# jhbastek/PhysicsInformedDiffusionModels

Hardware: AMD Instinct MI355X
Metric: training samples/sec (UNet+PDE-residual step), 64x64 Darcy (higher is better)
Workload: dtype f32

## Files before the change

### physicsinformeddiffusionmodels_amd/csrc/k_attn.hip

```cpp
#include "pidm_launch.h"

namespace pidm {

static const int DH = 32;

__device__ __forceinline__ float fexp(float x) { return __expf(x); }

__global__ void __launch_bounds__(256) la_kstats_kernel(const float* __restrict__ qkv, int N, int HD, int nseg,
                                                        float* __restrict__ kpart, float* __restrict__ kstat) {
  __shared__ float sm[4][64], ssum[4][64];
  const int b = blockIdx.y, seg = blockIdx.z, tid = threadIdx.x, cl = tid & 63, rl = tid >> 6;
  const int j = blockIdx.x * 64 + cl;
  const int per = (N + nseg - 1) / nseg;
  const int n_lo = seg * per, n_hi = (n_lo + per < N) ? n_lo + per : N;
  float m = -3.0e38f, s = 0.f;
  if (j < HD) {
    const float* base = qkv + (size_t)b * N * 3 * HD + HD + j;
    int n = n_lo + rl;
    for (; n + 28 < n_hi; n += 32) {
      float v[8];
#pragma unroll
      for (int u = 0; u < 8; ++u) v[u] = base[(size_t)(n + 4 * u) * 3 * HD];
      float gm = v[0];
#pragma unroll
// ... 950 lines not shown
    f32x16 acc;
    for (int r = 0; r < 16; ++r) acc[r] = 0.f;
#pragma unroll
    for (int s2 = 0; s2 < 16; ++s2)
      acc = __builtin_amdgcn_mfma_f32_32x32x2f32(sdo[32 * ti + l31][2 * s2 + half], sv[32 * tj + l31][2 * s2 + half], acc, 0, 0, 0);
#pragma unroll
    for (int r = 0; r < 16; ++r) sdS_[(32 * ti + (r & 3) + 8 * (r >> 2) + 4 * half) * LS + 32 * tj + l31] = acc[r];
  }
  if (wave < 2) {
    f32x16 acc;
    for (int r = 0; r < 16; ++r) acc[r] = 0.f;
#pragma unroll 8
    for (int s2 = 0; s2 < 32; ++s2)
      acc = __builtin_amdgcn_mfma_f32_32x32x2f32(sS_[(2 * s2 + half) * LS + 32 * wave + l31], sdo[2 * s2 + half][l31], acc, 0, 0, 0);
#pragma unroll
    for (int r = 0; r < 16; ++r)
      out[((size_t)b * N + 32 * wave + (r & 3) + 8 * (r >> 2) + 4 * half) * 3 * HD + 2 * HD + h * DH + l31] = acc[r];
  }
  __syncthreads();
  {
    const int row = tid >> 2, c0 = (tid & 3) * 16;
    const float* pp = sS_ + row * LS + c0;
    float* pd = sdS_ + row * LS + c0;
    float dot = 0.f;
#pragma unroll
    for (int j = 0; j < 16; ++j) dot = fmaf(pd[j], pp[j], dot);
    dot += pidm_quad_xor1(dot);
    dot += pidm_quad_xor2(dot);
#pragma unroll
    for (int j = 0; j < 16; ++j) pd[j] = pp[j] * (pd[j] - dot);
  }
  __syncthreads();
  {
    const int t = wave & 1;
    f32x16 acc;
    for (int r = 0; r < 16; ++r) acc[r] = 0.f;
    if (wave < 2) {
#pragma unroll 8
      for (int s2 = 0; s2 < 32; ++s2)
        acc = __builtin_amdgcn_mfma_f32_32x32x2f32(sdS_[(32 * t + l31) * LS + 2 * s2 + half], sk[2 * s2 + half][l31], acc, 0, 0, 0);
    } else {
#pragma unroll 8
      for (int s2 = 0; s2 < 32; ++s2)
        acc = __builtin_amdgcn_mfma_f32_32x32x2f32(sdS_[(2 * s2 + half) * LS + 32 * t + l31], sq[2 * s2 + half][l31], acc, 0, 0, 0);
    }
    const float f = wave < 2 ? scale : 1.f;
    const size_t col = (wave < 2 ? 0 : HD) + h * DH + l31;
#pragma unroll
    for (int r = 0; r < 16; ++r)
      out[((size_t)b * N + 32 * t + (r & 3) + 8 * (r >> 2) + 4 * half) * 3 * HD + col] = acc[r] * f;
  }
}

static int la_nsplit(int N) {
  int ns = N / 512;
  if (ns < 1) ns = 1;
  if (ns > 8) ns = 8;
  return ns;
}
static int la_kseg(int N) {
  int s = N / 256;
  if (s < 1) s = 1;
  if (s > 16) s = 16;
  return s;
}
size_t la_scratch_floats(int B, int N, int heads) {
  const size_t a = (size_t)B * la_kseg(N) * heads * DH * 2, b = (size_t)B * heads * la_nsplit(N) * 1024;
  return a + b + (size_t)heads * DH * 128 + 64;
}

int launch_la_forward(const float* qkv, float* kstat, float* ctx, float* attn, float* qstat, int B, int N, int heads,
                      float* scratch, hipStream_t st) {
  const int HD = heads * DH;
  const float scale = 0.17677669529663687f;
  const int nseg = la_kseg(N), NS = la_nsplit(N);
  float* kpart = scratch;
  float* dpart = scratch + (size_t)B * nseg * HD * 2;
  hipLaunchKernelGGL(la_kstats_kernel, dim3(cdiv(HD, 64), B, nseg), dim3(256), 0, st, qkv, N, HD, nseg, kpart, nseg == 1 ? kstat : nullptr);
  PIDM_CHECK_LAUNCH("la_kstats_kernel");
  if (nseg > 1) {
    hipLaunchKernelGGL(la_kstats_final_kernel, dim3(cdiv(B * HD, 256)), dim3(256), 0, st, kpart, B, HD, nseg, kstat);
    PIDM_CHECK_LAUNCH("la_kstats_final_kernel");
  }
  hipLaunchKernelGGL(HIP_KERNEL_NAME(la_nreduce_kernel<0>), dim3(B * heads, NS), dim3(256), 0, st, qkv, kstat, nullptr, nullptr,
                     dpart, N, heads, scale, NS == 1 ? ctx : nullptr, nullptr, 1.f / (float)N);
  PIDM_CHECK_LAUNCH("la_context");
  if (NS > 1) {
    hipLaunchKernelGGL(HIP_KERNEL_NAME(la_nreduce_final_kernel<0>), dim3(B * heads), dim3(256), 0, st, dpart, nullptr, ctx, nullptr, NS,
                       1.f / (float)N);
    PIDM_CHECK_LAUNCH("la_context_final");
  }
  const size_t npix = (size_t)B * N;
  if (N % 32 == 0)
    hipLaunchKernelGGL(HIP_KERNEL_NAME(la_out_kernel<true>), dim3((unsigned)((npix + 127) / 128), (npix + 127) / 128 < 1024 ? heads : 1), dim3(256), 0, st, qkv, ctx, attn,
                       qstat, N, heads, npix, scale);
  else
    hipLaunchKernelGGL(HIP_KERNEL_NAME(la_out_kernel<false>), dim3((unsigned)((npix + 127) / 128), (npix + 127) / 128 < 1024 ? heads : 1), dim3(256), 0, st, qkv, ctx, attn,
                       qstat, N, heads, npix, scale);
  PIDM_CHECK_LAUNCH("la_out_kernel");
  return 0;
}

int launch_la_backward(const float* qkv, const float* kstat, const float* qstat, const float* ctx, const float* dA, float* dctx,
                       float* rowdot, float* dqkv, int B, int N, int heads, float* scratch, hipStream_t st) {
  const float scale = 0.17677669529663687f;
  const int NS = la_nsplit(N);
  float* dpart = scratch;
  hipLaunchKernelGGL(HIP_KERNEL_NAME(la_nreduce_kernel<1>), dim3(B * heads, NS), dim3(256), 0, st, qkv, qstat, dA, ctx, dpart, N, heads,
                     scale, NS == 1 ? dctx : nullptr, rowdot, 1.f);
  PIDM_CHECK_LAUNCH("la_dctx");
  if (NS > 1) {
    hipLaunchKernelGGL(HIP_KERNEL_NAME(la_nreduce_final_kernel<1>), dim3(B * heads), dim3(256), 0, st, dpart, ctx, dctx, rowdot, NS, 1.f);
    PIDM_CHECK_LAUNCH("la_dctx_final");
  }
  if (N % 32 == 0 && N >= 64) {
    const size_t npix = (size_t)B * N;
    int ppb = N % 128 == 0 ? 128 : (N % 64 == 0 ? 64 : 32);
    (void)npix;
    if (const char* pe = knob("PIDM_LA_PPB")) { const int v = atoi(pe); if ((v == 32 || v == 64 || v == 128) && N % v == 0) ppb = v; }
    PIDM_PROF_NAME("la_bwd_pix_mfma_kernel");
    hipLaunchKernelGGL(la_bwd_pix_mfma_kernel, dim3((unsigned)((size_t)B * N / ppb), heads), dim3(2 * ppb), 0, st, qkv, kstat, qstat, ctx,
                       dctx, rowdot, dA, dqkv, N, heads, scale, ppb);
  } else {
    hipLaunchKernelGGL(la_bwd_pix_kernel, dim3(cdiv(N, 256), B * heads), dim3(256), 0, st, qkv, kstat, qstat, ctx, dctx, rowdot,
                       dA, dqkv, N, heads, scale);
  }
  PIDM_CHECK_LAUNCH("la_bwd_pix_kernel");
  return 0;
}

bool la_fused_ok(int N, int heads, int Cout, int ld_dy) {
  const bool off = knob("PIDM_NO_LA_FUSED") != nullptr;
  return !off && N % 128 == 0 && (Cout == 32 || Cout == 64 || Cout == 128) && (ld_dy & 3) == 0 && heads >= 1 && heads <= 14;
}
int launch_la_forward_fused(const float* qkv, float* kstat, float* ctx, float* qstat, const float* w_out, const float* bias,
                            const float* resid, float* y, int Cout, int B, int N, int heads, float* scratch, hipStream_t st) {
  if (!la_fused_ok(N, heads, Cout, Cout)) return fail("fused attention forward: N=%d Cout=%d not eligible", N, Cout);
  const int HD = heads * DH;
  const float scale = 0.17677669529663687f;
  const int nseg = la_kseg(N), NS = la_nsplit(N);
  float* kpart = scratch;
  float* dpart = scratch + (size_t)B * nseg * HD * 2;
  hipLaunchKernelGGL(la_kstats_kernel, dim3(cdiv(HD, 64), B, nseg), dim3(256), 0, st, qkv, N, HD, nseg, kpart, nseg == 1 ? kstat : nullptr);
  PIDM_CHECK_LAUNCH("la_kstats_kernel");
  if (nseg > 1) {
    hipLaunchKernelGGL(la_kstats_final_kernel, dim3(cdiv(B * HD, 256)), dim3(256), 0, st, kpart, B, HD, nseg, kstat);
    PIDM_CHECK_LAUNCH("la_kstats_final_kernel");
  }
  hipLaunchKernelGGL(HIP_KERNEL_NAME(la_nreduce_kernel<0>), dim3(B * heads, NS), dim3(256), 0, st, qkv, kstat, nullptr, nullptr,
                     dpart, N, heads, scale, NS == 1 ? ctx : nullptr, nullptr, 1.f / (float)N);
  PIDM_CHECK_LAUNCH("la_context");
  if (NS > 1) {
    hipLaunchKernelGGL(HIP_KERNEL_NAME(la_nreduce_final_kernel<0>), dim3(B * heads), dim3(256), 0, st, dpart, nullptr, ctx, nullptr, NS,
                       1.f / (float)N);
    PIDM_CHECK_LAUNCH("la_context_final");
  }
  float* wt = dpart + (size_t)B * heads * NS * 1024;
  hipLaunchKernelGGL(la_wt_kernel, dim3(cdiv(Cout * HD, 256)), dim3(256), 0, st, w_out, wt, Cout, HD);
// ... 44 lines not shown
    (void)hipFuncSetAttribute(reinterpret_cast<const void*>(&la_bwd_dkdv_kernel), hipFuncAttributeMaxDynamicSharedMemorySize, 96 * 1024);
    attr_done = true;
  }
  hipLaunchKernelGGL(la_bwd_dq_kernel, gridp, dim3(256), ((size_t)heads * 1056 + 4 * 32 * kLaTileLd) * sizeof(float), st, qkv, qstat, ctx, dy, ld_dy, w_out, Cout,
                     dqkv, N, heads, scale);
  PIDM_CHECK_LAUNCH("la_bwd_dq_kernel");
  hipLaunchKernelGGL(la_bwd_dkdv_kernel, gridp, dim3(256), ((size_t)heads * kLaDkvLds + 4 * 32 * kLaTileLd) * sizeof(float), st, qkv, kstat, dctx, rowdot, dqkv, N,
                     heads);
  PIDM_CHECK_LAUNCH("la_bwd_dkdv_kernel");
  return 0;
}

int launch_mid_attn(const float* qkv, const float* dO, float* out, int B, int N, int heads, bool bwd, hipStream_t st) {
  if (N > 64) return fail("mid attention: %d tokens > 64", N);
  const float scale = 0.17677669529663687f;
  const size_t lds = ((size_t)4 * N * 33 + (size_t)2 * N * (N + 1)) * sizeof(float);
  static bool attr_done = false;
  if (!attr_done) {
    (void)hipFuncSetAttribute(reinterpret_cast<const void*>(&mid_attn_kernel<true>), hipFuncAttributeMaxDynamicSharedMemorySize, 96 * 1024);
    (void)hipFuncSetAttribute(reinterpret_cast<const void*>(&mid_attn_kernel<false>), hipFuncAttributeMaxDynamicSharedMemorySize, 96 * 1024);
    attr_done = true;
  }
  const bool mfma_off = [] { const char* e = knob("PIDM_MID_ATTN_MFMA"); return e && !atoi(e); }();
  if (N == 64 && !mfma_off) {
    static bool attr64 = false;
    if (!attr64) {
      (void)hipFuncSetAttribute(reinterpret_cast<const void*>(&mid_attn64_kernel<true>), hipFuncAttributeMaxDynamicSharedMemorySize, 96 * 1024);
      (void)hipFuncSetAttribute(reinterpret_cast<const void*>(&mid_attn64_kernel<false>), hipFuncAttributeMaxDynamicSharedMemorySize, 96 * 1024);
      attr64 = true;
    }
    if (bwd) hipLaunchKernelGGL(HIP_KERNEL_NAME(mid_attn64_kernel<true>), dim3(B * heads), dim3(256), lds, st, qkv, dO, out, heads, scale);
    else hipLaunchKernelGGL(HIP_KERNEL_NAME(mid_attn64_kernel<false>), dim3(B * heads), dim3(256), lds, st, qkv, dO, out, heads, scale);
    PIDM_CHECK_LAUNCH("mid_attn64_kernel");
    return 0;
  }
  if (bwd)
    hipLaunchKernelGGL(HIP_KERNEL_NAME(mid_attn_kernel<true>), dim3(B * heads), dim3(256), lds, st, qkv, dO, out, N, heads, scale);
  else
    hipLaunchKernelGGL(HIP_KERNEL_NAME(mid_attn_kernel<false>), dim3(B * heads), dim3(256), lds, st, qkv, dO, out, N, heads, scale);
  PIDM_CHECK_LAUNCH("mid_attn_kernel");
  return 0;
}

}

extern "C" size_t pidm_linear_attention_ws(int B, int N, int heads) {
  return ((size_t)B * heads * (1024 + 32) + pidm::la_scratch_floats(B, N, heads)) * sizeof(float);
}
extern "C" int pidm_linear_attention_forward(const float* qkv, float* out, float* kstat, float* ctx, float* qstat, int B, int N,
                                             int heads, void* workspace, void* stream) {
  if (!qkv || !out || !kstat || !ctx || !qstat || !workspace || B < 1 || N < 1 || heads < 1)
    return pidm::fail("linear attention: bad arguments");
  float* scratch = reinterpret_cast<float*>(workspace) + (size_t)B * heads * (1024 + 32);
  return pidm::launch_la_forward(qkv, kstat, ctx, out, qstat, B, N, heads, scratch, reinterpret_cast<hipStream_t>(stream));
}
extern "C" int pidm_linear_attention_backward(const float* qkv, const float* kstat, const float* qstat, const float* ctx,
                                              const float* d_out, float* dqkv, int B, int N, int heads, void* workspace,
                                              void* stream) {
  if (!qkv || !kstat || !qstat || !ctx || !d_out || !dqkv || !workspace || B < 1 || N < 1 || heads < 1)
    return pidm::fail("linear attention backward: bad arguments");
  float* dctx = reinterpret_cast<float*>(workspace);
  float* rowdot = dctx + (size_t)B * heads * 1024;
  float* scratch = rowdot + (size_t)B * heads * 32;
  return pidm::launch_la_backward(qkv, kstat, qstat, ctx, d_out, dctx, rowdot, dqkv, B, N, heads, scratch,
                                  reinterpret_cast<hipStream_t>(stream));
}
extern "C" size_t pidm_linear_attention_out_backward_ws(int B, int N, int heads, int Cout) {
  return ((size_t)B * heads * (1024 + 32) + (size_t)B * Cout * heads * 32 + pidm::la_fused_scratch_floats(B, N, heads, Cout)) *
         sizeof(float);
}
extern "C" int pidm_linear_attention_out_backward(const float* qkv, const float* kstat, const float* qstat, const float* ctx,
                                                  const float* d_y, int ld_dy, const float* w_out, int Cout, float* dqkv,
                                                  float* dw_out, int B, int N, int heads, void* workspace, void* stream) {
  if (!qkv || !kstat || !qstat || !ctx || !d_y || !w_out || !dqkv || !dw_out || !workspace || B < 1)
    return pidm::fail("fused attention backward: bad arguments");
  const int HD = heads * 32;
  float* dctx = reinterpret_cast<float*>(workspace);
  float* rowdot = dctx + (size_t)B * heads * 1024;
  float* dwpart = rowdot + (size_t)B * heads * 32;
  float* scratch = dwpart + (size_t)B * Cout * HD;
  hipStream_t st = reinterpret_cast<hipStream_t>(stream);
  if (pidm::launch_la_backward_fused(qkv, kstat, qstat, ctx, d_y, ld_dy, w_out, Cout, dctx, rowdot, dqkv, dwpart, B, N, heads,
                                     scratch, st))
    return -1;
  return pidm::launch_split_reduce(dwpart, dw_out, nullptr, nullptr, B, Cout, HD, 1, Cout, HD, st);
}
extern "C" int pidm_linear_attention_out_forward(const float* qkv, const float* w_out, const float* bias, const float* residual,
                                                 float* y, int Cout, float* kstat, float* ctx, float* qstat, int B, int N,
                                                 int heads, void* workspace, void* stream) {
  if (!qkv || !w_out || !y || !kstat || !ctx || !qstat || !workspace || B < 1) return pidm::fail("fused attention forward: bad arguments");
  float* scratch = reinterpret_cast<float*>(workspace) + (size_t)B * heads * (1024 + 32);
  return pidm::launch_la_forward_fused(qkv, kstat, ctx, qstat, w_out, bias, residual, y, Cout, B, N, heads, scratch,
                                       reinterpret_cast<hipStream_t>(stream));
}
```

### physicsinformeddiffusionmodels_amd/csrc/pidm_launch.h

```cpp
#pragma once
#include <vector>

#include "pidm_common.h"

namespace pidm {
struct ReduceQueue {
  std::vector<ReduceDesc> v;
  unsigned nblocks = 0;
  void push(const float* src, float* dst, const float* bsrc, float* bdst, size_t sstride, int nsplit, int M, int N, int T,
            int MP, int NP) {
    ReduceDesc d{};
    d.src = src; d.dst = dst; d.bsrc = bsrc; d.bdst = bdst; d.sstride = sstride;
    d.nsplit = nsplit; d.M = M; d.N = N; d.T = T; d.MP = MP; d.NP = NP;
    const size_t total = (size_t)M * N * T + (bdst ? M : 0);
    const size_t flat = (size_t)MP * T * NP;
    d.blk0 = nblocks;
    d.mode = (nsplit <= 8 && T <= 16 && (size_t)M * N * T >= 32768) ? 1 : 0;
    if (d.mode == 0 && nsplit > 8 && flat >= 4096 && (flat & 3) == 0 && (sstride & 3) == 0 && (reinterpret_cast<size_t>(src) & 15) == 0) {
      d.mode = 2;
      d.bsrc = nullptr;
      d.bdst = nullptr;
      d.nblk = (unsigned)((flat / 4 + 31) / 32);
      nblocks += d.nblk;
      v.push_back(d);
// ... 70 lines not shown
bool conv_nt4_ok(const ConvGeom& g, int KC);
int launch_conv_rs(const ConvGeom& g, const float* src0, const float* src1, const unsigned short* wsplit, const float* bias,
                   const float* residual, float* out, hipStream_t st);
int launch_conv_fp32(const ConvGeom& g, const float* src0, const float* src1, const float* wp, const float* bias, const float* residual,
                     float* out, int sigmoid_last, hipStream_t st, int KC, int NT, bool nt4);
size_t packed_floats(const ConvGeom& g);
int packed_kp(const ConvGeom& g);
int launch_pack(const ConvGeom& g, int kind, const float* w_ref, float* w_packed, int srcKH, int srcKW, int n_off, int k_off,
                int n_src, int k_src, hipStream_t st);
unsigned make_pack_desc(const ConvGeom& g, int kind, const float* w_ref, float* w_packed, int srcKH, int srcKW, int n_off,
                        int k_off, int n_src, int k_src, PackDesc* d);
int launch_pack_multi(const PackDesc* table_dev, int ndesc, unsigned nblocks, hipStream_t st);
int launch_conv(const ConvGeom& g, const float* src0, const float* src1, const float* wp, const float* bias,
                const float* residual, float* out, int sigmoid_last, hipStream_t st);
size_t smallm_splitk_ws_floats(int M, int N, int K);
bool smallm_splitk_ok(int M, int N, int K, int lda, int ldw);
int launch_smallm_splitk(const float* A, int lda, const float* W, int ldw, float* out, int M, int N, int K, float* scratch, hipStream_t st);
size_t wgrad_ws_bytes(const ConvGeom& g);
int launch_wgrad(const ConvGeom& g, const float* src0, const float* src1, const float* dy, int ld_dy, float* dw_ref,
                 float* dbias, void* workspace, hipStream_t st, ReduceQueue* defer = nullptr, WgradQueue* wq = nullptr);
bool launch_wgrad_rs(const WgradGeom& plan, const float* src0, const float* src1, const float* dy, int ld_dy, float* partial,
                     float* bias_partial, hipStream_t st, WgradGeom* used, WgradQueue* wq = nullptr);
bool wgrad_rs_queueable(const ConvGeom& g, const float* src0, const float* dy, int ld_dy);
bool wgrad_rs4_eligible(const ConvGeom& g, int ld_dy);
bool launch_wgrad_rs4(const WgradGeom& plan, const float* src0, const float* src1, const float* dy, int ld_dy, float* partial,
                      float* bias_partial, hipStream_t st, WgradGeom* used, WgradQueue* wq = nullptr);
bool launch_wgrad_rs7(const WgradGeom& plan, const float* src0, const float* dy, int ld_dy, float* partial, float* bias_partial,
                      hipStream_t st, WgradGeom* used);
size_t colsum_ws_bytes(size_t rows, int C);
int launch_colsum(const float* x, size_t rows, int C, int ld, float* out, void* workspace, hipStream_t st,
                  ReduceQueue* defer = nullptr);
size_t gn_ws_bytes(int B, int HW, int C, int G);
int launch_gn_stats(const float* x, int B, int HW, int C, int G, float* stats, void* ws, hipStream_t st);
bool gn_apply_ln_ok(int C);
int launch_gn_apply(const float* x, float* stats, const float* gamma, const float* beta, const float* ss, const float* ssb,
                    int ldss, const float* res, float* y, int B, int HW, int C, int G, void* ws, hipStream_t st, int part_chunks = 0,
                    const float* ln_gamma = nullptr, float* ln_out = nullptr);
int launch_gn_bwd(const float* x, const float* dy, const float* stats, const float* gamma, const float* beta, const float* ss,
                  const float* ssb, int ldss, float* dss, float* dx, float* dgamma, float* dbeta, int B, int HW, int C, int G,
                  void* ws, hipStream_t st, float* dgb_persist = nullptr, ReduceQueue* defer = nullptr, int part_chunks = 0);
int launch_layernorm_fwd(const float* x, const float* gamma, float* y, size_t npix, int C, hipStream_t st);
size_t layernorm_bwd_ws_bytes(int C);
int layernorm_bwd_gn_chunks(int B, int HW);
int launch_layernorm_bwd(const float* x, const float* gamma, const float* dy, const float* res, float* dx, float* dgamma,
                         size_t npix, int C, void* ws, hipStream_t st, ReduceQueue* defer = nullptr, float* res_colsum = nullptr,
                         const float* gn_x = nullptr, const float* gn_stats = nullptr, const float* gn_gamma = nullptr,
                         const float* gn_beta = nullptr, int gn_G = 0, int gn_B = 0, int gn_HW = 0, void* gn_part = nullptr);
int launch_act_fwd(const float* x, float* y, size_t n, int act, hipStream_t st);
int launch_act_bwd(const float* x, const float* dy, float* dx, size_t n, int act, hipStream_t st);
int launch_sinusoid(const int64_t* t, float* emb, int B, int dim, hipStream_t st);
int launch_copy_add(float* dst, int ldd, const float* a, int lda, const float* b, int ldb, size_t rows, int cols, hipStream_t st);
int launch_nchw_to_nhwc(const float* src, float* dst, int B, int C, int HW, const float* y_sig, hipStream_t st);
size_t la_scratch_floats(int B, int N, int heads);
int launch_la_forward(const float* qkv, float* kstat, float* ctx, float* attn, float* qstat, int B, int N, int heads,
                      float* scratch, hipStream_t st);
bool la_fused_ok(int N, int heads, int Cout, int ld_dy);
bool la_fused_pays(int B, int N);
size_t la_fused_scratch_floats(int B, int N, int heads, int Cout);
int launch_la_forward_fused(const float* qkv, float* kstat, float* ctx, float* qstat, const float* w_out, const float* bias,
                            const float* resid, float* y, int Cout, int B, int N, int heads, float* scratch, hipStream_t st);
int launch_la_backward_fused(const float* qkv, const float* kstat, const float* qstat, const float* ctx, const float* dy, int ld_dy,
                             const float* w_out, int Cout, float* dctx, float* rowdot, float* dqkv, float* dwpart, int B, int N,
                             int heads, float* scratch, hipStream_t st);
int launch_la_backward(const float* qkv, const float* kstat, const float* qstat, const float* ctx, const float* dA, float* dctx,
                       float* rowdot, float* dqkv, int B, int N, int heads, float* scratch, hipStream_t st);
bool lap_ok(int N, int heads, int C, int Cout);
size_t lap_scratch_floats(int B, int N, int heads, int C);
size_t lap_saved_floats(int B, int heads, int C);
size_t lap_dw_ranges(int N, int C);
size_t lap_bwd_tmp_floats(int B, int heads, int C);
int launch_lap_forward(const float* xn, const float* wqkv, const float* wout, const float* bias, const float* resid, float* y,
                       float* saved, float* qstat, int C, int B, int N, int heads, float* scratch, hipStream_t st);
int launch_lap_backward(const float* xn, const float* dy, const float* wqkv, const float* wout, const float* saved, const float* qstat,
                        float* dxn, float* dwqk_part, float* dwv_part, float* dwout_part, float* tmp, int C, int B, int N, int heads,
                        float* scratch, hipStream_t st);
int launch_mid_attn(const float* qkv, const float* dO, float* out, int B, int N, int heads, bool bwd, hipStream_t st);
}
```

### physicsinformeddiffusionmodels_amd/csrc/unet_engine.hip

```cpp
#include <map>
#include <string>
#include <vector>

#include <stdlib.h>

#include "pidm_launch.h"

extern char** environ;

namespace pidm {

struct Arena {
  char* base = nullptr;
  size_t off = 0, hwm = 0, cap = 0;
  bool dry = false;
  float* alloc(size_t nfloats) {
    off = align_up(off, 256);
    char* p = base + off;
    off += nfloats * sizeof(float);
    if (off > hwm) hwm = off;
    return reinterpret_cast<float*>(p);
  }
  size_t mark() const { return off; }
  void release(size_t m) { off = m; }
  bool overflow() const { return !dry && hwm > cap; }
};

struct ConvLayer {
  int w = -1, b = -1;
  int C0 = 0, C1 = 0, Cout = 0, K = 1, stride = 1, pad = 0, transposed = 0, H = 1;
  size_t off_f = 0, off_d = 0;
  bool dgrad = true;
  int pad_mode = 0;
};

struct ResBlock {
  ConvLayer c1, c2, cr;
  bool has_mlp = false, has_res = false;
  int C0 = 0, C1 = 0, Co = 0, H = 0;
  int gn1w = -1, gn1b = -1, gn2w = -1, gn2b = -1, mlpw = -1, mlpb = -1;
  int ss_off = 0;
  const float *x0 = nullptr, *x1 = nullptr;
  float *a = nullptr, *st1 = nullptr, *bact = nullptr, *c = nullptr, *st2 = nullptr;
};

struct AttnBlock {
  bool mid = false;
  int C = 0, H = 0, gamma = -1;
  ConvLayer qkv, out;
  const float* x = nullptr;
  float *xn = nullptr, *qkvb = nullptr, *kstat = nullptr, *qstat = nullptr, *ctx = nullptr, *attn = nullptr;
  bool xn_ready = false;
  float* out_pre = nullptr;
  size_t mk_pre = 0;
  float* lsaved = nullptr;
  bool projected = false;
};

struct GraphSeg {
  hipGraph_t graph = nullptr;
  hipGraphExec_t exec = nullptr;
  hipEvent_t ev_after = nullptr;
  long long kernels = 0;
};
struct TapeState {
  std::vector<ResBlock> rb;
  std::vector<AttnBlock> attn;
  std::vector<const float*> skip, down_in, up_in;
  int tape_B = 0;
  const float* x_in = nullptr;
  float *emb = nullptr, *h1 = nullptr, *h1g = nullptr, *temb = nullptr, *st = nullptr, *ss = nullptr, *h0 = nullptr, *xfinal = nullptr;
  const float* out_nchw = nullptr;
  bool tape_cond = false;
  const float* cond_in = nullptr;
  float *e1 = nullptr, *e1g = nullptr, *e2 = nullptr, *h0pre = nullptr;
  int plan_B = 0;
  size_t plan_tape_b = 0, plan_tmp_b = 0, plan_defer_b = 0;
};
struct GraphEntry {
  std::vector<uint64_t> key;
  std::vector<GraphSeg> segs;
  TapeState tape;
  const void* red_dev = nullptr;
  uint64_t stamp = 0;
};
struct GraphCapture {
  GraphEntry* entry = nullptr;
  hipStream_t user_st = nullptr;
  bool open = false, failed = false;
  long long kernels0 = 0;
};
static const size_t kMaxGraphs = 6;
static const size_t kMaxSeenKeys = 16;
static long long g_graph_launches = 0, g_graph_kernels = 0, g_graph_captures = 0;
static void graph_entry_free(GraphEntry& e) {
  for (auto& sg : e.segs) {
    if (sg.exec) (void)hipGraphExecDestroy(sg.exec);
    if (sg.graph) (void)hipGraphDestroy(sg.graph);
  }
  e.segs.clear();
}

}

using namespace pidm;

struct pidm_unet {
  pidm_unet_cfg cfg;
  std::vector<std::string> names;
// ... 578 lines not shown
         7919L * (wgrad_group_on(1, 1, false) ? 1 : 0) +
         104729L * (knob("PIDM_WGRAD_GROUP_MAXWORK") ? atol(knob("PIDM_WGRAD_GROUP_MAXWORK")) % 65521 : 0) +
         15485863L * (knob("PIDM_LAP_NPER_DIV") ? atol(knob("PIDM_LAP_NPER_DIV")) % 8 : 0);
}
static bool attn_shape_projectable(const AttnBlock& a, int heads) { return !a.mid && a.out.b >= 0 && lap_ok(a.H * a.H, heads, a.C, a.C); }
static bool attn_projected(const AttnBlock& a, int heads) {
  bool off; int min_n;
  lap_knobs(&off, &min_n);
  return !off && a.H * a.H >= min_n && attn_shape_projectable(a, heads);
}

static int attn_fwd(Run& r, AttnBlock& a, const float* x, float** out_p) {
  pidm_unet* U = r.U;
  const int B = r.B, N = a.H * a.H, C = a.C, heads = U->heads, HD = heads * 32;
  const size_t npix = (size_t)B * N;
  float* out = a.xn_ready ? a.out_pre : act_alloc(r, npix * C);
  const size_t mk = a.xn_ready ? a.mk_pre : r.tmp.mark();
  a.x = x;
  if (!a.xn_ready) {
    a.xn = act_alloc(r, npix * C);
    RUN(launch_layernorm_fwd(x, U->P[a.gamma], a.xn, npix, C, r.st));
  }
  a.xn_ready = false;
  a.projected = attn_projected(a, heads);
  if (a.projected) {
    a.qkvb = nullptr;
    a.lsaved = act_alloc(r, lap_saved_floats(B, heads, C));
    a.qstat = act_alloc(r, npix * heads * 2);
    RUN(launch_lap_forward(a.xn, U->P[a.qkv.w], U->P[a.out.w], U->P[a.out.b], x, out, a.lsaved, a.qstat, C, B, N, heads, r.scratch, r.st));
    r.tmp.release(mk);
    *out_p = out;
    return 0;
  }
  a.qkvb = act_alloc(r, npix * 3 * HD);
  if (conv_fwd(r, a.qkv, a.xn, nullptr, nullptr, a.qkvb)) return -1;
  if (!a.mid && (la_fused_ok(N, heads, C, C) && la_fused_pays(B, N))) {
    a.attn = nullptr;
    a.kstat = act_alloc(r, (size_t)B * HD * 2);
    a.ctx = act_alloc(r, (size_t)B * heads * 1024);
    a.qstat = act_alloc(r, npix * heads * 2);
    RUN(launch_la_forward_fused(a.qkvb, a.kstat, a.ctx, a.qstat, U->P[a.out.w], a.out.b >= 0 ? U->P[a.out.b] : nullptr, x, out, C, B,
                                N, heads, r.scratch, r.st));
    r.tmp.release(mk);
    *out_p = out;
    return 0;
  }
  a.attn = act_alloc(r, npix * HD);
  if (a.mid) {
    RUN(launch_mid_attn(a.qkvb, nullptr, a.attn, B, N, heads, false, r.st));
  } else {
    a.kstat = act_alloc(r, (size_t)B * HD * 2);
    a.ctx = act_alloc(r, (size_t)B * heads * 1024);
    a.qstat = act_alloc(r, npix * heads * 2);
    RUN(launch_la_forward(a.qkvb, a.kstat, a.ctx, a.attn, a.qstat, B, N, heads, r.scratch, r.st));
  }
  if (conv_fwd(r, a.out, a.attn, nullptr, x, out)) return -1;
  r.tmp.release(mk);
  *out_p = out;
  return 0;
}

static int forward_impl(Run& r, const float* x_nhwc, const int64_t* t, float* out_nchw, const float* cond_nhwc) {
  pidm_unet* U = r.U;
  const int B = r.B, P = U->cfg.image_size, dim = U->cfg.dim, n = U->n_lv, td = U->tdim;
  U->tape_B = B;
  U->x_in = x_nhwc;
  U->out_nchw = out_nchw;
  U->emb = act_alloc(r, (size_t)B * dim);
  RUN(launch_sinusoid(t, U->emb, B, dim, r.st));
  U->h1 = act_alloc(r, (size_t)B * td);
  if (conv_fwd(r, U->lin1, U->emb, nullptr, nullptr, U->h1)) return -1;
  U->h1g = act_alloc(r, (size_t)B * td);
  RUN(launch_act_fwd(U->h1, U->h1g, (size_t)B * td, 1, r.st));
  U->temb = act_alloc(r, (size_t)B * td);
  if (conv_fwd(r, U->lin2, U->h1g, nullptr, nullptr, U->temb)) return -1;
  U->st = act_alloc(r, (size_t)B * td);
  RUN(launch_act_fwd(U->temb, U->st, (size_t)B * td, 0, r.st));
  U->ss = act_alloc(r, (size_t)B * U->ss_total);
  if (conv_fwd(r, U->lincat, U->st, nullptr, nullptr, U->ss)) return -1;

  U->h0 = act_alloc(r, (size_t)B * P * P * dim);
  if (conv_fwd(r, U->init_conv, x_nhwc, nullptr, nullptr, U->h0)) return -1;
  U->tape_cond = cond_nhwc != nullptr;
  if (cond_nhwc) {
    const size_t nh = (size_t)B * P * P * dim;
    U->cond_in = cond_nhwc;
    U->h0pre = U->h0;
    U->e1 = act_alloc(r, nh);
    if (conv_fwd(r, U->emb1, cond_nhwc, nullptr, nullptr, U->e1)) return -1;
    U->e1g = act_alloc(r, nh);
    RUN(launch_act_fwd(U->e1, U->e1g, nh, 1, r.st));
    U->e2 = act_alloc(r, nh);
    if (conv_fwd(r, U->emb2, U->e1g, nullptr, nullptr, U->e2)) return -1;
    float* hc = act_alloc(r, nh);
    if (conv_fwd(r, U->comb, U->h0pre, U->e2, nullptr, hc)) return -1;
    U->h0 = hc;
  }
  float* x = U->h0;
  int irb = 0, iat = 0;
  for (int i = 0; i < n; ++i) {
    if (resblock_fwd(r, U->rb[irb++], x, nullptr, &x)) return -1;
    if (resblock_fwd(r, U->rb[irb++], x, nullptr, &x, &U->attn[iat])) return -1;
    if (attn_fwd(r, U->attn[iat++], x, &x)) return -1;
    U->skip[i] = x;
    if (i < n - 1) {
      U->down_in[i] = x;
      const int Ho = out_h(U->down[i]);
// ... 220 lines not shown
  if (r.dry ? attn_projected(a, heads) : a.projected) {
    const size_t nr = (size_t)B * lap_dw_ranges(N, C);
    const size_t n_qk = nr * 2 * HD * C, n_v = (size_t)B * HD * C, n_o = (size_t)B * C * HD;
    float* dwqk = r.defer_on ? r.defer.alloc(n_qk) : r.tmp.alloc(n_qk);
    float* dwv = r.defer_on ? r.defer.alloc(n_v) : r.tmp.alloc(n_v);
    float* dwo = r.defer_on ? r.defer.alloc(n_o) : r.tmp.alloc(n_o);
    float* ltmp = r.tmp.alloc(lap_bwd_tmp_floats(B, heads, C));
    g_xn = r.tmp.alloc(npix * C);
    RUN(launch_lap_backward(a.xn, g_out, U->P[a.qkv.w], U->P[a.out.w], a.lsaved, a.qstat, g_xn, dwqk, dwv, dwo, ltmp, C, B, N, heads, r.scratch,
                            r.st));
    if (U->have_grads && !r.dry) {
      float* gw = U->G[a.qkv.w];
      if (r.q()) {
        r.q()->push(dwqk, gw, nullptr, nullptr, (size_t)2 * HD * C, (int)nr, 2 * HD, C, 1, 2 * HD, C);
        r.q()->push(dwv, gw + (size_t)2 * HD * C, nullptr, nullptr, (size_t)HD * C, B, HD, C, 1, HD, C);
        r.q()->push(dwo, U->G[a.out.w], nullptr, nullptr, (size_t)C * HD, B, C, HD, 1, C, HD);
      } else {
        RUN(launch_split_reduce(dwqk, gw, nullptr, nullptr, (int)nr, 2 * HD, C, 1, 2 * HD, C, r.st));
        RUN(launch_split_reduce(dwv, gw + (size_t)2 * HD * C, nullptr, nullptr, B, HD, C, 1, HD, C, r.st));
        RUN(launch_split_reduce(dwo, U->G[a.out.w], nullptr, nullptr, B, C, HD, 1, C, HD, r.st));
      }
    }
    float* ln_part = r.part_alloc(layernorm_bwd_ws_bytes(C) + colsum_ws_bytes(1024, C));
    RUN(launch_layernorm_bwd(a.x, U->P[a.gamma], g_xn, g_out, g_x, U->G[a.gamma], npix, C, ln_part, r.st, r.q(),
                             (U->have_grads && !r.dry) ? U->G[a.out.b] : nullptr, gn_x, gn_st, gn_gm, gn_bt, U->groups, B, N, gn_part));
    if (pc_prev) *pc_prev = gn_pc;
    if (!r.keep_frames()) r.tmp.release(mk);
    return 0;
  }
  if (!a.mid && (la_fused_ok(N, heads, C, C) && la_fused_pays(B, N))) {
    g_qkv = r.tmp.alloc(npix * 3 * HD);
    float* dctx = r.tmp.alloc((size_t)B * heads * 1024);
    float* rowdot = r.tmp.alloc((size_t)B * heads * 32);
    const size_t dwn = (size_t)B * C * HD;
    float* dwpart = r.defer_on ? r.defer.alloc(dwn) : r.tmp.alloc(dwn);
    RUN(launch_la_backward_fused(a.qkvb, a.kstat, a.qstat, a.ctx, g_out, C, U->P[a.out.w], C, dctx, rowdot, g_qkv, dwpart, B, N,
                                 heads, r.scratch, r.st));
    if (U->have_grads && !r.dry) {
      if (r.q()) r.q()->push(dwpart, U->G[a.out.w], nullptr, nullptr, (size_t)C * HD, B, C, HD, 1, C, HD);
      else RUN(launch_split_reduce(dwpart, U->G[a.out.w], nullptr, nullptr, B, C, HD, 1, C, HD, r.st));
      if (a.out.b >= 0) out_bias_with_ln = true;
    }
    g_xn = r.tmp.alloc(npix * C);
  } else {
    if (conv_wgrad(r, a.out, a.attn, nullptr, g_out)) return -1;
    float* g_attn = r.tmp.alloc(npix * HD);
    if (conv_dgrad(r, a.out, g_out, nullptr, g_attn)) return -1;
    g_qkv = r.tmp.alloc(npix * 3 * HD);
    if (a.mid) {
      RUN(launch_mid_attn(a.qkvb, g_attn, g_qkv, B, N, heads, true, r.st));
    } else {
      float* dctx = r.tmp.alloc((size_t)B * heads * 1024);
      float* rowdot = r.tmp.alloc((size_t)B * heads * 32);
      RUN(launch_la_backward(a.qkvb, a.kstat, a.qstat, a.ctx, g_attn, dctx, rowdot, g_qkv, B, N, heads, r.scratch, r.st));
    }
    g_xn = g_attn;
    if (C > HD) g_xn = r.tmp.alloc(npix * C);
  }
  if (conv_wgrad(r, a.qkv, a.xn, nullptr, g_qkv)) return -1;
  if (conv_dgrad(r, a.qkv, g_qkv, nullptr, g_xn)) return -1;
  float* ln_part = r.part_alloc(layernorm_bwd_ws_bytes(C) + colsum_ws_bytes(1024, C));
  RUN(launch_layernorm_bwd(a.x, U->P[a.gamma], g_xn, g_out, g_x, U->G[a.gamma], npix, C, ln_part, r.st, r.q(),
                           out_bias_with_ln ? U->G[a.out.b] : nullptr, gn_x, gn_st, gn_gm, gn_bt, U->groups, B, N, gn_part));
  if (pc_prev) *pc_prev = gn_pc;
  if (!r.keep_frames()) r.tmp.release(mk);
  return 0;
}

static size_t scratch_floats_needed(pidm_unet* U, int B) {
  size_t mx = 1 << 16;
  auto upd = [&](size_t bytes) { if (bytes / 4 + 64 > mx) mx = bytes / 4 + 64; };
  auto conv_ws = [&](const ConvLayer& L) {
    ConvGeom g;
    if (L.transposed) {
      if (geom_wgrad_transposed(L, B, L.Cout, &g)) return;
    } else if (geom_fwd_layer(L, B, 0, &g)) {
      return;
    }
    upd(wgrad_ws_bytes(g));
    const int Ho = out_h(L);
    upd(colsum_ws_bytes((size_t)B * Ho * Ho, L.Cout));
  };
  conv_ws(U->init_conv); conv_ws(U->lin1); conv_ws(U->lin2); conv_ws(U->lincat); conv_ws(U->final_conv);
  for (auto& m : U->rb) {
    conv_ws(m.c1); conv_ws(m.c2);
    if (m.has_res) conv_ws(m.cr);
    upd(gn_ws_bytes(B, m.H * m.H, m.Co, U->groups));
  }
  for (auto& a : U->attn) {
    conv_ws(a.qkv); conv_ws(a.out);
    upd(layernorm_bwd_ws_bytes(a.C) + colsum_ws_bytes(1024, a.C));
    upd(la_scratch_floats(B, a.H * a.H, U->heads) * sizeof(float));
    if (attn_shape_projectable(a, U->heads)) upd(lap_scratch_floats(B, a.H * a.H, U->heads, a.C) * sizeof(float));
    if (!a.mid && la_fused_ok(a.H * a.H, U->heads, a.C, a.C) && la_fused_pays(B, a.H * a.H)) upd(la_fused_scratch_floats(B, a.H * a.H, U->heads, a.C) * sizeof(float));
  }
  for (int i = 0; i < U->n_lv - 1; ++i) { conv_ws(U->down[i]); conv_ws(U->up[i]); }
  return mx;
}

static int cap_begin(Run& r) {
  GraphCapture* c = r.cap;
  if (hipStreamBeginCapture(r.st, hipStreamCaptureModeThreadLocal) != hipSuccess) {
    (void)hipGetLastError();
    c->failed = true;
    return fail("graph capture: hipStreamBeginCapture failed");
  }
  c->open = true;
// ... 676 lines not shown
```

Baseline: 8228.

## Add single-block-per-head linear attention forward and backward kernels for small N

```diff
diff --git a/physicsinformeddiffusionmodels_amd/csrc/k_attn.hip b/physicsinformeddiffusionmodels_amd/csrc/k_attn.hip
--- a/physicsinformeddiffusionmodels_amd/csrc/k_attn.hip
+++ b/physicsinformeddiffusionmodels_amd/csrc/k_attn.hip
@@ -1026,6 +1026,255 @@
   }
 }
 
+template <int NT>
+__global__ void __launch_bounds__(256) la_one_fwd_kernel(const float* __restrict__ qkv, float* __restrict__ out,
+                                                         float* __restrict__ kstat, float* __restrict__ ctx,
+                                                         float* __restrict__ qstat, int heads, float scale) {
+  constexpr int N = 32 * NT, PW = 4 * NT;
+  __shared__ float red[4][1024], sc[32][33], smax[4][32];
+  __shared__ double ssum[8][32];
+  const int bh = blockIdx.x, b = bh / heads, h = bh % heads, HD = heads * DH;
+  const int tid = threadIdx.x, lane = tid & 63, half = lane >> 5, l31 = lane & 31;
+  const int wave = __builtin_amdgcn_readfirstlane(tid >> 6);
+  const float* q0 = qkv + (size_t)b * N * 3 * HD + h * DH;
+  float kx[PW], vx[PW];
+  {
+    const float* kp = q0 + (size_t)(wave * 2 * PW + half) * 3 * HD + HD + l31;
+#pragma unroll
+    for (int j = 0; j < PW; ++j) {
+      kx[j] = kp[(size_t)(2 * j) * 3 * HD];
+      vx[j] = kp[(size_t)(2 * j) * 3 * HD + HD];
+    }
+  }
+  f32x4 qn[4] = {};
+  if (wave < NT) {
+    const float* qp = q0 + (size_t)(32 * wave + l31) * 3 * HD + 16 * half;
+#pragma unroll
+    for (int k = 0; k < 4; ++k) qn[k] = *reinterpret_cast<const f32x4*>(qp + 4 * k);
+  }
+  float m = kx[0];
+#pragma unroll
+  for (int j = 1; j < PW; ++j) m = fmaxf(m, kx[j]);
+  m = fmaxf(m, pidm_other_half(m));
+  if (half == 0) smax[wave][l31] = m;
+  __syncthreads();
+  const float cm = fmaxf(fmaxf(smax[0][l31], smax[1][l31]), fmaxf(smax[2][l31], smax[3][l31]));
+  double s = 0.0;
+#pragma unroll
+  for (int j = 0; j < PW; ++j) {
+    kx[j] = fexp(kx[j] - cm);
+    s += (double)kx[j];
+  }
+  ssum[2 * wave + half][l31] = s;
+  __syncthreads();
+  double S = ssum[0][l31];
+#pragma unroll
+  for (int w = 1; w < 8; ++w) S += ssum[w][l31];
+  const float cis = 1.f / (float)S;
+  if (wave == 0 && half == 0) {
+    kstat[((size_t)b * HD + h * DH + l31) * 2] = cm;
+    kstat[((size_t)b * HD + h * DH + l31) * 2 + 1] = cis;
+  }
+  f32x16 acc;
+  for (int r = 0; r < 16; ++r) acc[r] = 0.f;
+#pragma unroll
+  for (int j = 0; j < PW; ++j) acc = __builtin_amdgcn_mfma_f32_32x32x2f32(kx[j] * cis, vx[j], acc, 0, 0, 0);
+#pragma unroll
+  for (int r = 0; r < 16; ++r) red[wave][((r & 3) + 8 * (r >> 2) + 4 * half) * 32 + l31] = acc[r];
+  __syncthreads();
+  {
+    const float alpha = 1.f / (float)N;
+#pragma unroll
+    for (int k = 0; k < 4; ++k) {
+      const int e = tid + 256 * k;
+      const float v = ((red[0][e] + red[1][e]) + (red[2][e] + red[3][e])) * alpha;
+      ctx[(size_t)bh * 1024 + e] = v;
+      sc[e >> 5][e & 31] = v;
+    }
+  }
+  __syncthreads();
+  for (int t = wave; t < NT; t += 4) {
+    float qv[16];
+#pragma unroll
+    for (int k = 0; k < 4; ++k) { qv[4 * k] = qn[k][0]; qv[4 * k + 1] = qn[k][1]; qv[4 * k + 2] = qn[k][2]; qv[4 * k + 3] = qn[k][3]; }
+    if (t + 4 < NT) {
+      const float* qp = q0 + (size_t)(32 * (t + 4) + l31) * 3 * HD + 16 * half;
+#pragma unroll
+      for (int k = 0; k < 4; ++k) qn[k] = *reinterpret_cast<const f32x4*>(qp + 4 * k);
+    }
+    float qm = qv[0];
+#pragma unroll
+    for (int k = 1; k < 16; ++k) qm = fmaxf(qm, qv[k]);
+    qm = fmaxf(qm, pidm_other_half(qm));
+    float qs = 0.f;
+#pragma unroll
+    for (int k = 0; k < 16; ++k) {
+      qv[k] = fexp(qv[k] - qm);
+      qs += qv[k];
+    }
+    qs += pidm_other_half(qs);
+    const float inv = 1.f / qs;
+    const size_t p = (size_t)b * N + 32 * t + l31;
+    if (half == 0) *reinterpret_cast<float2*>(qstat + (p * heads + h) * 2) = make_float2(qm, inv);
+    f32x16 o;
+    for (int r = 0; r < 16; ++r) o[r] = 0.f;
+#pragma unroll
+    for (int s2 = 0; s2 < 16; ++s2) o = __builtin_amdgcn_mfma_f32_32x32x2f32(qv[s2] * inv * scale, sc[16 * half + s2][l31], o, 0, 0, 0);
+    float* ob = out + ((size_t)b * N + 32 * t) * HD + h * DH + l31;
+#pragma unroll
+    for (int r = 0; r < 16; ++r) ob[(size_t)((r & 3) + 8 * (r >> 2) + 4 * half) * HD] = o[r];
+  }
+}
+
+static const int kLaOneLd = 33;
+static size_t la_one_bwd_lds(int N) { return ((size_t)4 * N * kLaOneLd + 2 * 32 * kLaOneLd + 4096 + 32) * sizeof(float); }
+
+template <int UNR>
+__device__ __forceinline__ void la_one_stage(const float* __restrict__ qrow, const float* __restrict__ drow,
+                                             const float* __restrict__ srow, int HD, int heads, int lq, int ld, int ls, float km,
+                                             float kis, float scale, float* __restrict__ sq, float* __restrict__ sp,
+                                             float* __restrict__ sv, float* __restrict__ sda, int lo, f32x16& acc) {
+  float qa[UNR], ka[UNR], va[UNR], da[UNR];
+  float2 st[UNR];
+#pragma unroll
+  for (int u = 0; u < UNR; ++u) {
+    const float* r = qrow + (size_t)(2 * u) * 3 * HD;
+    qa[u] = r[lq];
+    ka[u] = r[lq + HD];
+    va[u] = r[lq + 2 * HD];
+    da[u] = (drow + (size_t)(2 * u) * HD)[ld];
+    st[u] = *reinterpret_cast<const float2*>(srow + (size_t)(2 * u) * heads * 2 + ls);
+  }
+#pragma unroll
+  for (int u = 0; u < UNR; ++u) {
+    const float qs = fexp(qa[u] - st[u].x) * st[u].y;
+    const int o = lo + 2 * u * kLaOneLd;
+    sq[o] = qs;
+    sp[o] = fexp(ka[u] - km) * kis;
+    sv[o] = va[u];
+    sda[o] = da[u];
+    acc = __builtin_amdgcn_mfma_f32_32x32x2f32(qs * scale, da[u], acc, 0, 0, 0);
+  }
+}
+
+template <int NW>
+__global__ void __launch_bounds__(64 * NW) la_one_bwd_kernel(const float* __restrict__ qkv, const float* __restrict__ kstat,
+                                                             const float* __restrict__ qstat, const float* __restrict__ ctx,
+                                                             const float* __restrict__ dA, float* __restrict__ dqkv, int N, int heads,
+                                                             float scale) {
+  HIP_DYNAMIC_SHARED(float, sm)
+  constexpr int LS = kLaOneLd, NTH = 64 * NW, EPT = 1024 / NTH;
+  float* sq = sm;
+  float* sp = sq + (size_t)N * LS;
+  float* sv = sp + (size_t)N * LS;
+  float* sda = sv + (size_t)N * LS;
+  float* sc = sda + (size_t)N * LS;
+  float* sd = sc + 32 * LS;
+  float* red = sd + 32 * LS;
+  float* srd = red + 4096;
+  const int bh = blockIdx.x, b = bh / heads, h = bh % heads, HD = heads * DH;
+  const int tid = threadIdx.x, lane = tid & 63, half = lane >> 5, l31 = lane & 31;
+  const int wave = __builtin_amdgcn_readfirstlane(tid >> 6);
+  float cv[EPT];
+#pragma unroll
+  for (int k = 0; k < EPT; ++k) cv[k] = ctx[(size_t)bh * 1024 + tid + NTH * k];
+  const float km = kstat[((size_t)b * HD + h * DH + l31) * 2], kis = kstat[((size_t)b * HD + h * DH + l31) * 2 + 1];
+  f32x16 acc;
+  for (int r = 0; r < 16; ++r) acc[r] = 0.f;
+  {
+    const int per = N / NW, n_lo = wave * per;
+    const int lq = half * 3 * HD + h * DH + l31, ld = half * HD + h * DH + l31, ls = (half * heads + h) * 2;
+    int n0 = n_lo;
+    if (NW == 8)
+      for (; n0 + 32 <= n_lo + per; n0 += 32)
+        la_one_stage<16>(qkv + ((size_t)b * N + n0) * 3 * HD, dA + ((size_t)b * N + n0) * HD, qstat + ((size_t)b * N + n0) * heads * 2, HD,
+                         heads, lq, ld, ls, km, kis, scale, sq, sp, sv, sda, (n0 + half) * LS + l31, acc);
+    for (; n0 + 16 <= n_lo + per; n0 += 16)
+      la_one_stage<8>(qkv + ((size_t)b * N + n0) * 3 * HD, dA + ((size_t)b * N + n0) * HD, qstat + ((size_t)b * N + n0) * heads * 2, HD,
+                      heads, lq, ld, ls, km, kis, scale, sq, sp, sv, sda, (n0 + half) * LS + l31, acc);
+    if (n0 < n_lo + per)
+      la_one_stage<4>(qkv + ((size_t)b * N + n0) * 3 * HD, dA + ((size_t)b * N + n0) * HD, qstat + ((size_t)b * N + n0) * heads * 2, HD,
+                      heads, lq, ld, ls, km, kis, scale, sq, sp, sv, sda, (n0 + half) * LS + l31, acc);
+  }
+  if (NW == 8) {
+    if (wave >= 4) {
+#pragma unroll
+      for (int r = 0; r < 16; ++r) red[(wave - 4) * 1024 + ((r & 3) + 8 * (r >> 2) + 4 * half) * 32 + l31] = acc[r];
+    }
+    __syncthreads();
+    if (wave < 4) {
+#pragma unroll
+      for (int r = 0; r < 16; ++r) acc[r] += red[wave * 1024 + ((r & 3) + 8 * (r >> 2) + 4 * half) * 32 + l31];
+    }
+  }
+  if (wave < 4) {
+#pragma unroll
+    for (int r = 0; r < 16; ++r) red[wave * 1024 + ((r & 3) + 8 * (r >> 2) + 4 * half) * 32 + l31] = acc[r];
+  }
+#pragma unroll
+  for (int k = 0; k < EPT; ++k) sc[((tid + NTH * k) >> 5) * LS + (tid & 31)] = cv[k];
+  __syncthreads();
+  float dv4[EPT];
+#pragma unroll
+  for (int k = 0; k < EPT; ++k) {
+    const int e = tid + NTH * k;
+    dv4[k] = (red[e] + red[1024 + e]) + (red[2048 + e] + red[3072 + e]);
+  }
+  __syncthreads();
+#pragma unroll
+  for (int k = 0; k < EPT; ++k) {
+    const int e = tid + NTH * k, o = (e >> 5) * LS + (e & 31);
+    sd[o] = dv4[k];
+    red[o] = dv4[k] * cv[k];
+  }
+  __syncthreads();
+  if (tid < 32) {
+    float sacc = 0.f;
+    for (int j = 0; j < 32; ++j) sacc += red[tid * LS + j];
+    srd[tid] = sacc;
+  }
+  __syncthreads();
+  const float invN = 1.f / (float)N, rd = srd[l31];
+  for (int it = wave, turn = 0; it < N / 16; it += NW, ++turn) {
+    const int t = it >> 1;
+    const bool part_dq = ((wave ^ (wave >> 2) ^ turn) & 1) == 0;
+    const int ra = (32 * t + l31) * LS + 16 * half;
+    float* ob = dqkv + ((size_t)b * N + 32 * t) * 3 * HD + h * DH + l31;
+    if (part_dq) {
+      f32x16 acc1;
+      for (int r = 0; r < 16; ++r) acc1[r] = 0.f;
+#pragma unroll
+      for (int s = 0; s < 16; ++s)
+        acc1 = __builtin_amdgcn_mfma_f32_32x32x2f32(sda[ra + s], sc[l31 * LS + 16 * half + s], acc1, 0, 0, 0);
+#pragma unroll
+      for (int r = 0; r < 16; ++r) {
+        const int row = (r & 3) + 8 * (r >> 2) + 4 * half;
+        const float qs = sq[(32 * t + row) * LS + l31];
+        float dot = qs * acc1[r];
+#pragma unroll
+        for (int off = 1; off < 32; off <<= 1) dot += __shfl_xor(dot, off);
+        ob[(size_t)row * 3 * HD] = scale * qs * (acc1[r] - dot);
+      }
+    } else {
+      f32x16 acc2, acc3;
+      for (int r = 0; r < 16; ++r) { acc2[r] = 0.f; acc3[r] = 0.f; }
+#pragma unroll
+      for (int s = 0; s < 16; ++s) {
+        const int kk = 16 * half + s;
+        acc2 = __builtin_amdgcn_mfma_f32_32x32x2f32(sv[ra + s], sd[l31 * LS + kk], acc2, 0, 0, 0);
+        acc3 = __builtin_amdgcn_mfma_f32_32x32x2f32(sp[ra + s], sd[kk * LS + l31], acc3, 0, 0, 0);
+      }
+#pragma unroll
+      for (int r = 0; r < 16; ++r) {
+        const int row = (r & 3) + 8 * (r >> 2) + 4 * half;
+        float* o = ob + (size_t)row * 3 * HD;
+        o[HD] = sp[(32 * t + row) * LS + l31] * (acc2[r] * invN - rd);
+        o[2 * HD] = acc3[r] * invN;
+      }
+    }
+  }
+}
+
 static int la_nsplit(int N) {
   int ns = N / 512;
   if (ns < 1) ns = 1;
@@ -1043,10 +1292,33 @@
   return a + b + (size_t)heads * DH * 128 + 64;
 }
 
+static bool la_one_pays(int B, int N) {
+  (void)B; (void)N;
+  return true;
+}
+bool la_one_on(int B, int N) {
+  const char* e = knob("PIDM_LA_ONE");
+  if (e && !atoi(e)) return false;
+  return N >= 32 && N <= 256 && N % 32 == 0 && la_one_pays(B, N);
+}
+
 int launch_la_forward(const float* qkv, float* kstat, float* ctx, float* attn, float* qstat, int B, int N, int heads,
-                      float* scratch, hipStream_t st) {
+                      float* scratch, hipStream_t st, bool one) {
   const int HD = heads * DH;
   const float scale = 0.17677669529663687f;
+  if (one) {
+    if (N < 32 || N > 256 || N % 32) return fail("one-launch attention forward: N=%d not eligible", N);
+    const dim3 grid(B * heads), blk(256);
+#define PIDM_LA_ONE_FWD(NT_) \
+  case NT_: hipLaunchKernelGGL(HIP_KERNEL_NAME(la_one_fwd_kernel<NT_>), grid, blk, 0, st, qkv, attn, kstat, ctx, qstat, heads, scale); break;
+    switch (N / 32) {
+      PIDM_LA_ONE_FWD(1) PIDM_LA_ONE_FWD(2) PIDM_LA_ONE_FWD(3) PIDM_LA_ONE_FWD(4)
+      PIDM_LA_ONE_FWD(5) PIDM_LA_ONE_FWD(6) PIDM_LA_ONE_FWD(7) PIDM_LA_ONE_FWD(8)
+    }
+#undef PIDM_LA_ONE_FWD
+    PIDM_CHECK_LAUNCH("la_one_fwd_kernel");
+    return 0;
+  }
   const int nseg = la_kseg(N), NS = la_nsplit(N);
   float* kpart = scratch;
   float* dpart = scratch + (size_t)B * nseg * HD * 2;
@@ -1076,8 +1348,28 @@
 }
 
 int launch_la_backward(const float* qkv, const float* kstat, const float* qstat, const float* ctx, const float* dA, float* dctx,
-                       float* rowdot, float* dqkv, int B, int N, int heads, float* scratch, hipStream_t st) {
+                       float* rowdot, float* dqkv, int B, int N, int heads, float* scratch, hipStream_t st, bool one) {
   const float scale = 0.17677669529663687f;
+  if (one) {
+    if (N < 32 || N > 256 || N % 32) return fail("one-launch attention backward: N=%d not eligible", N);
+    static bool attr_done = false;
+    if (!attr_done) {
+      if (hipFuncSetAttribute(reinterpret_cast<const void*>(&la_one_bwd_kernel<8>), hipFuncAttributeMaxDynamicSharedMemorySize,
+                              (int)la_one_bwd_lds(256)) != hipSuccess ||
+          hipFuncSetAttribute(reinterpret_cast<const void*>(&la_one_bwd_kernel<4>), hipFuncAttributeMaxDynamicSharedMemorySize,
+                              (int)la_one_bwd_lds(224)) != hipSuccess)
+        return fail("one-launch attention backward: %zu bytes of LDS not granted", la_one_bwd_lds(256));
+      attr_done = true;
+    }
+    if (N >= 128 && N % 64 == 0)
+      hipLaunchKernelGGL(HIP_KERNEL_NAME(la_one_bwd_kernel<8>), dim3(B * heads), dim3(512), la_one_bwd_lds(N), st, qkv, kstat, qstat, ctx,
+                         dA, dqkv, N, heads, scale);
+    else
+      hipLaunchKernelGGL(HIP_KERNEL_NAME(la_one_bwd_kernel<4>), dim3(B * heads), dim3(256), la_one_bwd_lds(N), st, qkv, kstat, qstat, ctx,
+                         dA, dqkv, N, heads, scale);
+    PIDM_CHECK_LAUNCH("la_one_bwd_kernel");
+    return 0;
+  }
   const int NS = la_nsplit(N);
   float* dpart = scratch;
   hipLaunchKernelGGL(HIP_KERNEL_NAME(la_nreduce_kernel<1>), dim3(B * heads, NS), dim3(256), 0, st, qkv, qstat, dA, ctx, dpart, N, heads,
@@ -1228,7 +1520,8 @@
   if (!qkv || !out || !kstat || !ctx || !qstat || !workspace || B < 1 || N < 1 || heads < 1)
     return pidm::fail("linear attention: bad arguments");
   float* scratch = reinterpret_cast<float*>(workspace) + (size_t)B * heads * (1024 + 32);
-  return pidm::launch_la_forward(qkv, kstat, ctx, out, qstat, B, N, heads, scratch, reinterpret_cast<hipStream_t>(stream));
+  return pidm::launch_la_forward(qkv, kstat, ctx, out, qstat, B, N, heads, scratch, reinterpret_cast<hipStream_t>(stream),
+                                 pidm::la_one_on(B, N));
 }
 extern "C" int pidm_linear_attention_backward(const float* qkv, const float* kstat, const float* qstat, const float* ctx,
                                               const float* d_out, float* dqkv, int B, int N, int heads, void* workspace,
@@ -1239,7 +1532,7 @@
   float* rowdot = dctx + (size_t)B * heads * 1024;
   float* scratch = rowdot + (size_t)B * heads * 32;
   return pidm::launch_la_backward(qkv, kstat, qstat, ctx, d_out, dctx, rowdot, dqkv, B, N, heads, scratch,
-                                  reinterpret_cast<hipStream_t>(stream));
+                                  reinterpret_cast<hipStream_t>(stream), pidm::la_one_on(B, N));
 }
 extern "C" size_t pidm_linear_attention_out_backward_ws(int B, int N, int heads, int Cout) {
   return ((size_t)B * heads * (1024 + 32) + (size_t)B * Cout * heads * 32 + pidm::la_fused_scratch_floats(B, N, heads, Cout)) *
diff --git a/physicsinformeddiffusionmodels_amd/csrc/pidm_launch.h b/physicsinformeddiffusionmodels_amd/csrc/pidm_launch.h
--- a/physicsinformeddiffusionmodels_amd/csrc/pidm_launch.h
+++ b/physicsinformeddiffusionmodels_amd/csrc/pidm_launch.h
@@ -146,8 +146,9 @@
 int launch_copy_add(float* dst, int ldd, const float* a, int lda, const float* b, int ldb, size_t rows, int cols, hipStream_t st);
 int launch_nchw_to_nhwc(const float* src, float* dst, int B, int C, int HW, const float* y_sig, hipStream_t st);
 size_t la_scratch_floats(int B, int N, int heads);
+bool la_one_on(int B, int N);
 int launch_la_forward(const float* qkv, float* kstat, float* ctx, float* attn, float* qstat, int B, int N, int heads,
-                      float* scratch, hipStream_t st);
+                      float* scratch, hipStream_t st, bool one);
 bool la_fused_ok(int N, int heads, int Cout, int ld_dy);
 bool la_fused_pays(int B, int N);
 size_t la_fused_scratch_floats(int B, int N, int heads, int Cout);
@@ -157,7 +158,7 @@
                              const float* w_out, int Cout, float* dctx, float* rowdot, float* dqkv, float* dwpart, int B, int N,
                              int heads, float* scratch, hipStream_t st);
 int launch_la_backward(const float* qkv, const float* kstat, const float* qstat, const float* ctx, const float* dA, float* dctx,
-                       float* rowdot, float* dqkv, int B, int N, int heads, float* scratch, hipStream_t st);
+                       float* rowdot, float* dqkv, int B, int N, int heads, float* scratch, hipStream_t st, bool one);
 bool lap_ok(int N, int heads, int C, int Cout);
 size_t lap_scratch_floats(int B, int N, int heads, int C);
 size_t lap_saved_floats(int B, int heads, int C);
diff --git a/physicsinformeddiffusionmodels_amd/csrc/unet_engine.hip b/physicsinformeddiffusionmodels_amd/csrc/unet_engine.hip
--- a/physicsinformeddiffusionmodels_amd/csrc/unet_engine.hip
+++ b/physicsinformeddiffusionmodels_amd/csrc/unet_engine.hip
@@ -55,6 +55,7 @@
   size_t mk_pre = 0;
   float* lsaved = nullptr;
   bool projected = false;
+  bool la_one = false;
 };
 
 struct GraphSeg {
@@ -739,7 +740,8 @@
     a.kstat = act_alloc(r, (size_t)B * HD * 2);
     a.ctx = act_alloc(r, (size_t)B * heads * 1024);
     a.qstat = act_alloc(r, npix * heads * 2);
-    RUN(launch_la_forward(a.qkvb, a.kstat, a.ctx, a.attn, a.qstat, B, N, heads, r.scratch, r.st));
+    a.la_one = la_one_on(B, N);
+    RUN(launch_la_forward(a.qkvb, a.kstat, a.ctx, a.attn, a.qstat, B, N, heads, r.scratch, r.st, a.la_one));
   }
   if (conv_fwd(r, a.out, a.attn, nullptr, x, out)) return -1;
   r.tmp.release(mk);
@@ -1066,7 +1068,7 @@
     } else {
       float* dctx = r.tmp.alloc((size_t)B * heads * 1024);
       float* rowdot = r.tmp.alloc((size_t)B * heads * 32);
-      RUN(launch_la_backward(a.qkvb, a.kstat, a.qstat, a.ctx, g_attn, dctx, rowdot, g_qkv, B, N, heads, r.scratch, r.st));
+      RUN(launch_la_backward(a.qkvb, a.kstat, a.qstat, a.ctx, g_attn, dctx, rowdot, g_qkv, B, N, heads, r.scratch, r.st, a.la_one));
     }
     g_xn = g_attn;
     if (C > HD) g_xn = r.tmp.alloc(npix * C);
```

Result: no change. 8290 (median of 6 runs) (+0.7%).
